# mikeferguson/ndt_2d

Measured on AMD Instinct MI355X. Metric: pose-candidates x beams scored per second, higher is better.
Workload: dtype f64

## Files before the change

### ndt_2d_amd/csrc/ndt2d_device_fn.h

```cpp
#ifndef NDT2D_DEVICE_FN_H_
#define NDT2D_DEVICE_FN_H_

#include <hip/hip_runtime.h>
#include <math.h>

#include "ndt2d_kernels.h"

namespace ndt2d
{

constexpr int kWave = 64;
constexpr int kRecord = 12;
constexpr double kNoIndex = 1.0e308;
constexpr double kPadCoord = -1.0e300;

template <bool POW2>
__device__ __forceinline__ uint32_t cell_index(const GridDesc & g, double px, double py)
{
  const double tx = px - g.origin_x;
  const double ty = py - g.origin_y;
  double fx, fy;
  if (POW2)
  {
    fx = tx * g.inv_cell_size;
// ... 8 lines not shown
                      (fy < static_cast<double>(g.size_y));
  const uint32_t gx = static_cast<uint32_t>(fx);
  const uint32_t gy = static_cast<uint32_t>(fy);
  return inside ? gy * g.size_x + gx : g.ncell;
}

__device__ __forceinline__ double record_exponent(double mx, double my, double h00,
                                                  double h01, double h11, double px, double py)
{
  const double q0 = px - mx;
  const double q1 = py - my;
  const double r0 = q0 * h00 + q1 * h01;
  const double r1 = q0 * h01 + q1 * h11;
  return r0 * q0 + r1 * q1;
}

__device__ __forceinline__ double record_likelihood(double mx, double my, double h00,
                                                    double h01, double h11, double px,
                                                    double py)
{
  return exp(record_exponent(mx, my, h00, h01, h11, px, py));
}

__device__ __forceinline__ double fma3(double a, double b, double c)
{
  double d;
  asm("v_fma_f64 %0, %1, %2, %3" : "=v"(d) : "v"(a), "v"(b), "v"(c));
  return d;
}
#ifndef NDT2D_EXP_SCALAR_CONSTANTS
#define NDT2D_EXP_SCALAR_CONSTANTS 0
#endif
template <uint32_t HI, uint32_t LO>
__device__ __forceinline__ double fma3k(double a, double b)
{
  double d;
#if NDT2D_EXP_SCALAR_CONSTANTS
  uint32_t lo, hi;
  asm volatile("s_mov_b32 %0, %2\n\ts_mov_b32 %1, %3" : "=s"(lo), "=s"(hi) : "n"(LO), "n"(HI));
  const double c = __hiloint2double(static_cast<int>(hi), static_cast<int>(lo));
  asm("v_fma_f64 %0, %1, %2, %3" : "=v"(d) : "v"(a), "v"(b), "s"(c));
#else
  asm("v_fma_f64 %0, %1, %2, %3" : "=v"(d) : "v"(a), "v"(b), "v"(__hiloint2double(static_cast<int>(HI), static_cast<int>(LO))));
#endif
  return d;
}

__device__ __forceinline__ double exp_of_exponent(double x)
{
  asm("v_max_f64 %0, %1, %2" : "=v"(x) : "v"(x), "s"(-1000.0));
  const double n = rint(x * 1.4426950408889634);
  double r = fma(n, -0.6931471805599453, x);
  r = fma(n, -2.3190468138462996e-17, r);
  double p = fma3k<0x3e928af3u, 0xfca7ab0cu>(r, 0x1.ade156a5dcb37p-26);
  p = fma3k<0x3ec71deeu, 0x623fde64u>(r, p);
  p = fma3k<0x3efa0199u, 0x7c89e6b0u>(r, p);
  p = fma3k<0x3f2a01a0u, 0x14761f6eu>(r, p);
  p = fma3k<0x3f56c16cu, 0x1852b7b0u>(r, p);
  p = fma3k<0x3f811111u, 0x11122322u>(r, p);
  p = fma3k<0x3fa55555u, 0x555502a1u>(r, p);
  p = fma3k<0x3fc55555u, 0x55555511u>(r, p);
  p = fma3k<0x3fe00000u, 0x0000000bu>(r, p);
  asm("v_fma_f64 %0, %1, %2, 1.0" : "=v"(p) : "v"(r), "v"(p));
  asm("v_fma_f64 %0, %1, %2, 1.0" : "=v"(p) : "v"(r), "v"(p));
  return ldexp(p, static_cast<int>(n));
}

__device__ __forceinline__ bool wave_any(bool p)
{
  return __builtin_amdgcn_ballot_w64(p) != 0ull;
}

constexpr double kExpOverflowAbove = 0x1.62e42fefa39efp+9;

__device__ __forceinline__ double exp_score(double e)
{
  double r = exp_of_exponent(e);
  if (__builtin_expect(wave_any(!(e <= kExpOverflowAbove)), 0))
  {
    r = (e != e) ? e + e : (e > kExpOverflowAbove ? HUGE_VAL : r);
  }
  return r;
}

__device__ __forceinline__ double negligible_below(double s)
{
  const double from_sum =
// ... 179 lines not shown
```

### ndt_2d_amd/csrc/ndt2d_lane_fn.h

```cpp
#ifndef NDT2D_LANE_FN_H_
#define NDT2D_LANE_FN_H_

#include <cmath>

#include "ndt2d_device_fn.h"

namespace ndt2d
{

namespace
{

constexpr int kPatch = 8;
#ifndef NDT2D_LANE_UNROLL
#define NDT2D_LANE_UNROLL 8
#endif
constexpr int kUnroll = NDT2D_LANE_UNROLL;
constexpr double kFracScale = 65536.0;
constexpr int kMapStride = 256;
constexpr int kMaxMapCells = 256;
constexpr uint32_t kNearUnits = 4;
constexpr double kBoxMargin = 1.0 / 1024.0;
constexpr double kTwo24 = 16777216.0;
constexpr double kTwo52 = 4503599627370496.0;
// ... 193 lines not shown
  return kRankLead + (((ncell + 1u) * 2u + 15u) & ~15u);
}

#if defined(NDT2D_LANE_HIST) || defined(NDT2D_LANE_PATHS)
__device__ double * g_lane_hist = nullptr;
#endif
#ifdef NDT2D_LANE_PATHS
#define NDT2D_PATH(slot, amount)                                                              \
  do {                                                                                        \
    if (g_lane_hist != nullptr && (threadIdx.x & 63u) == 0) atomicAdd(g_lane_hist + (slot), static_cast<double>(amount)); \
  } while (0)
#else
#define NDT2D_PATH(slot, amount) do {} while (0)
#endif

struct LaneCtx
{
  uint32_t rank_address;
  uint32_t lds_cells_address;
  uint32_t sub_log2;
  uint32_t exact_index;
  uint32_t idx_bias;
  uint32_t size_x;
};

__device__ __forceinline__ uint32_t lds_byte_at(uint32_t address)
{
  typedef const __attribute__((address_space(3))) uint8_t * lds_byte_ptr;
  return *reinterpret_cast<lds_byte_ptr>(address);
}

__device__ __forceinline__ uint32_t lds_u16_at(uint32_t address)
{
  typedef const __attribute__((address_space(3))) uint16_t * lds_u16_ptr;
  return *reinterpret_cast<lds_u16_ptr>(address);
}

__device__ __forceinline__ uint64_t near_boundary(uint32_t v)
{
  uint64_t lanes;
  asm("v_cmp_gt_u16_e64 %0, 8, %1" : "=s"(lanes) : "v"(v));
  return lanes;
}

__device__ __forceinline__ uint2 lds_two_dwords_at(uint32_t address)
{
  typedef const __attribute__((address_space(3), aligned(4))) uint32_t * lds_u32_ptr;
// ... 32 lines not shown
}

struct SkipState
{
  double skip_below;
  uint32_t skip_level;
};

__device__ __forceinline__ SkipState skip_state(double sum, int32_t no_skip)
{
  SkipState s;
  if (no_skip)
  {
    s.skip_below = -HUGE_VAL;
    s.skip_level = 0;
    return s;
  }
  s.skip_below = negligible_below(sum);
  const int32_t l = static_cast<int32_t>(ceil(s.skip_below)) + 63;
  s.skip_level = static_cast<uint32_t>(min(max(l, 1), 63)) << 2;
  return s;
}

template <int U, bool POW2, bool LDS_RECORDS, bool SCALAR_ROWS = true, bool COMPACT = false>
__device__ __forceinline__ void lane_beams(const GridDesc & g, const LaneCtx & c,
                                           const double4 (&o)[U], double dx, double dy,
                                           double dxy, double & sum, SkipState & skip,
                                           int32_t no_skip)
{
  const double skip_below = skip.skip_below;
  const uint32_t skip_level = skip.skip_level;
  uint32_t lo[U], hi[U], m[U];
  uint32_t top = 0;
#pragma unroll
  for (int u = 0; u < U; ++u)
  {
    const double s = o[u].z + dxy;
    lo[u] = static_cast<uint32_t>(__double2loint(s));
    hi[u] = static_cast<uint32_t>(__double2hiint(s));
    m[u] = lds_byte_at(__builtin_amdgcn_perm(hi[u], lo[u], 0x0c0c0502u));
    top = max(top, m[u]);
  }
  NDT2D_PATH(U == 1 ? 210 : 202, U);
  if (wave_any(top >= skip_level))
  {
    NDT2D_PATH(203, 1);
    bool added = false;
    if (SCALAR_ROWS)
    {
#pragma unroll
      for (int u = 0; u < U; ++u) asm volatile("" : : "s"(o[u].x), "s"(o[u].y));
    }
#pragma unroll
    for (int u = 0; u < U; ++u)
    {
      const uint64_t live_mask = __builtin_amdgcn_ballot_w64(m[u] >= skip_level);
      if (live_mask != 0ull)
      {
        NDT2D_PATH(204, 1);
        const uint32_t fy = __builtin_amdgcn_perm(hi[u], lo[u], 0x0c0c0403u);
        const bool occ = (m[u] & 1u) != 0;
        const uint64_t near_mask =
          (near_boundary(lo[u]) | near_boundary(fy) | ((no_skip | c.exact_index) != 0 ? ~0ull : 0ull)) & live_mask;
        const uint64_t occ_lanes = __builtin_amdgcn_ballot_w64(occ);
        const uint64_t occ_mask = occ_lanes & live_mask;
#ifdef NDT2D_LANE_NO_EXACT
        if ((occ_mask | near_mask) == 0x1234567ull)
#else
        if ((occ_mask | near_mask) != 0ull)
#endif
        {
          NDT2D_PATH(205, 1);
          if (near_mask != 0ull) NDT2D_PATH(206, 1);
          const double px = o[u].x + dx;
          const double py = o[u].y + dy;
          uint32_t idx;
          if (near_mask != 0ull)
          {
            idx = cell_index<POW2>(g, px, py);
          }
          else
          {
            const uint32_t col = ((lo[u] >> 16) & 0xffu) >> c.sub_log2;
            const uint32_t row = ((hi[u] >> 8) & 0xffu) >> c.sub_log2;
            const uint32_t cell = __umul24(row, c.size_x) + (col - c.idx_bias);
            if (COMPACT)
            {
              asm("v_cndmask_b32 %0, -1, %1, %2" : "=v"(idx) : "v"(cell), "s"(occ_lanes));
            }
            else
            {
              idx = occ ? cell : g.ncell;
            }
          }
          if (COMPACT) idx = lds_u16_at(c.rank_address + 2u * idx);
          const double e = LDS_RECORDS ? lds_record_exponent(c.lds_cells_address, idx, px, py)
                                       : indexed_exponent<false>(g, nullptr, idx, px, py);
#ifdef NDT2D_LANE_HIST
          if (g_lane_hist != nullptr)
          {
            const uint64_t flagged = occ_mask | near_mask;
            const uint64_t needed = __builtin_amdgcn_ballot_w64(!(e < skip_below)) & flagged;
            if ((threadIdx.x & 63u) == 0)
            {
              atomicAdd(g_lane_hist + __popcll(flagged), 1.0);
              atomicAdd(g_lane_hist + 70 + __popcll(needed), 1.0);
              atomicAdd(g_lane_hist + (needed != 0ull ? 140 : 141), 1.0);
            }
          }
#endif
          if (wave_any(!(e < skip_below)))
          {
            NDT2D_PATH(207, 1);
            sum += exp_score(e);
            added = true;
          }
        }
      }
// ... 99 lines not shown
```

### ndt_2d_amd/csrc/ndt2d_match_lane.hip

```cpp
#include <cmath>
#include <cstdlib>

#include <type_traits>

#include "ndt2d_lane_fn.h"

namespace ndt2d
{

namespace
{

constexpr uint32_t kDynamicItemsFromBeams = 256;
constexpr int kLaneThreads = 1024;
constexpr int kLaneThreadsSmall = 256;
#ifndef NDT2D_LANE_THREADS_COMPACT
#define NDT2D_LANE_THREADS_COMPACT 768
#endif
constexpr int kLaneThreadsCompact = NDT2D_LANE_THREADS_COMPACT;
#define NDT2D_LANE_COMPACT_WAVES_PER_EU (NDT2D_LANE_THREADS_COMPACT / 128)

__global__ void __launch_bounds__(256) outer_table_kernel(const MatchArgs a, double4 * outer,
                                                          uint8_t * map_out, const LaneGeom geo)
{
  {
    const GridDesc & g = a.grid;
    const uint32_t n_map = static_cast<uint32_t>(kMapStride) * geo.map_h;
    for (uint32_t i = blockIdx.x * 256 + threadIdx.x; i < n_map; i += gridDim.x * 256)
    {
      const int32_t mx = static_cast<int32_t>(i & (kMapStride - 1));
      const int32_t my = static_cast<int32_t>(i >> 8);
      if (geo.block_log2 > 0)
      {
        const int32_t cells = 1 << geo.block_log2;
        map_out[i] = block_byte(g, mx * cells - geo.pad + geo.win_x0, my * cells - geo.pad + geo.win_y0, cells);
        continue;
      }
      const int32_t sub = 1 << geo.sub_log2;
      const int32_t cx = (mx >> geo.sub_log2) - geo.pad + geo.win_x0;
      const int32_t cy = (my >> geo.sub_log2) - geo.pad + geo.win_y0;
      map_out[i] = sub_cell_byte(g, cx, cy, mx & (sub - 1), my & (sub - 1), geo.sub_log2);
    }
  }

  if (blockIdx.x == 0 && threadIdx.x < kItemShards) a.next_item[threadIdx.x * kItemShardStride] = 0u;
  const uint64_t n = static_cast<uint64_t>(a.th_end - a.th_begin) * a.n_beams;
  for (uint64_t i = static_cast<uint64_t>(blockIdx.x) * 256 + threadIdx.x; i < n;
       i += static_cast<uint64_t>(gridDim.x) * 256)
  {
    const uint32_t t = static_cast<uint32_t>(i / a.n_beams);
    const uint32_t b = static_cast<uint32_t>(i - static_cast<uint64_t>(t) * a.n_beams);
    const uint32_t ith = a.th_begin + t * a.th_stride;
    const double ct = a.cos_th[ith];
    const double st = a.sin_th[ith];
    const double2 p = reinterpret_cast<const double2 *>(a.beams_xy)[b];
    double4 o;
    o.x = p.x * ct - p.y * st + a.pose_x;
    o.y = p.x * st + p.y * ct + a.pose_y;
    double kx = ((o.x - a.grid.origin_x) * a.grid.inv_cell_size + (geo.pad - geo.win_x0)) * geo.unit_scale;
    double ky = ((o.y - a.grid.origin_y) * a.grid.inv_cell_size + (geo.pad - geo.win_y0)) * geo.unit_scale;
    kx = !(kx >= geo.k_min) ? geo.k_min : (kx > geo.k_max_x ? geo.k_max_x : kx);
    ky = !(ky >= geo.k_min) ? geo.k_min : (ky > geo.k_max_y ? geo.k_max_y : ky);
    o.z = kTwo52 + (rint(ky) * kTwo24 + rint(kx)) + kNearBias;
    o.w = 0.0;
    outer[i] = o;
  }
}

__device__ __forceinline__ void item_place(uint32_t item, uint32_t patches, uint32_t patches_1d,
                                           uint32_t th_mid, uint32_t & t, uint32_t & pxi, uint32_t & pyi)
{
  const uint32_t rank = item / patches;
  const uint32_t p = item - rank * patches;
  t = (rank & 1u) ? th_mid + (rank + 1u) / 2u : th_mid - rank / 2u;
  pxi = p / patches_1d;
  pyi = p - pxi * patches_1d;
}

__device__ __forceinline__ double packed_offset(double dx, double dy, double inv_scaled)
{
  return rint(dy * inv_scaled) * kTwo24 + rint(dx * inv_scaled);
}

__device__ __forceinline__ double no_index_here()
{
  static_assert(kNoIndex == 1.0e308, "the literal below is 1.0e308");
  uint32_t lo, hi;
  asm volatile("v_mov_b32 %0, 0x85ebc8a0\n\tv_mov_b32 %1, 0x7fe1ccf3" : "=v"(lo), "=v"(hi));
  return __hiloint2double(static_cast<int>(hi), static_cast<int>(lo));
}

template <int THREADS, bool POW2, bool LDS_RECORDS, bool DYNAMIC_ITEMS, bool COMPACT, bool PARTS = false>
__device__ __forceinline__ void match_lane_body(
  const MatchArgs & a, const double4 * __restrict__ outer, const uint8_t * __restrict__ map_image,
  const LaneGeom & geo)
{
  extern __shared__ __align__(16) double lds[];
  const GridDesc & g = a.grid;
#if defined(NDT2D_LANE_HIST) || defined(NDT2D_LANE_PATHS)
  if (blockIdx.x == 0 && threadIdx.x == 0) g_lane_hist = a.scores;
#endif
  uint8_t * lds_map = reinterpret_cast<uint8_t *>(lds);
  const uint32_t map_bytes = static_cast<uint32_t>(geo.map_h) * kMapStride;
  const uint32_t rank_bytes = COMPACT ? compact_rank_bytes(g.ncell) : 0u;
  double * lds_cells = lds + (map_bytes + rank_bytes) / sizeof(double);

  if (COMPACT)
  {
    const uint4 * src_rank = reinterpret_cast<const uint4 *>(g.cell_rank);
    uint4 * dst_rank = reinterpret_cast<uint4 *>(lds_map + map_bytes + kRankLead);
    for (uint32_t i = threadIdx.x; i < (rank_bytes - kRankLead) / 16; i += THREADS) dst_rank[i] = src_rank[i];
    if (threadIdx.x == 0)
    {
      reinterpret_cast<uint16_t *>(lds_map + map_bytes + kRankLead)[-1] = static_cast<uint16_t>(g.n_occ);
    }
    const uint32_t n2 = (g.n_occ + 1) * kCellDoubles / 2;
    const double2 * src = reinterpret_cast<const double2 *>(g.compact_records);
// ... 5 lines not shown
    stage_grid_to_lds(g, lds_cells);
  }
  {
    const uint32_t n16 = static_cast<uint32_t>(kMapStride) * geo.map_h / 16;
    const uint4 * src = reinterpret_cast<const uint4 *>(map_image);
    uint4 * dst = reinterpret_cast<uint4 *>(lds_map);
    for (uint32_t i = threadIdx.x; i < n16; i += THREADS) dst[i] = src[i];
  }
  __syncthreads();

#ifdef NDT2D_LANE_TRACE
  const unsigned long long trace_t0 = wall_clock64();
  unsigned long long trace_last = trace_t0, trace_max = 0, trace_last_start = trace_t0;
  uint32_t trace_items = 0, trace_prev_item = 0, trace_flagged = 0;
#endif
  LaneCtx c;
  c.rank_address = map_bytes + (COMPACT ? kRankLead : 0u);
  c.lds_cells_address = map_bytes + rank_bytes;
  c.sub_log2 = static_cast<uint32_t>(geo.sub_log2);
  c.exact_index = geo.block_log2 > 0 ? 1u : 0u;
  c.idx_bias = static_cast<uint32_t>(geo.pad - geo.win_y0) * g.size_x +
               static_cast<uint32_t>(geo.pad - geo.win_x0);
  c.size_x = g.size_x;

  const uint32_t lane = threadIdx.x & (kWave - 1);
  const uint32_t wave = __builtin_amdgcn_readfirstlane(threadIdx.x >> 6);
  const uint32_t n_lin = a.n_lin;
  const uint32_t patches_1d = (n_lin + kPatch - 1) / kPatch;
  const uint32_t patches = patches_1d * patches_1d;
  const uint32_t n_items = (a.th_end - a.th_begin) * patches * (PARTS ? a.beam_parts : 1u);
  constexpr uint32_t kLaneWaves = THREADS / kWave;
  const uint32_t n_workers = gridDim.x * kLaneWaves;
  const uint32_t worker = wave * gridDim.x + blockIdx.x;
  const uint64_t per_theta = static_cast<uint64_t>(n_lin) * n_lin;
  const uint32_t th_mid = (a.th_end - a.th_begin - 1u) / 2u;
  const uint32_t home_shard = blockIdx.x % kItemShards;
  const double inv_scaled = geo.inv_scaled;

  double best_s = 0.0;
  double best_i = kNoIndex;
  double acc[10];
#pragma unroll
  for (int k = 0; k < 10; ++k) acc[k] = 0.0;
  for (uint32_t item = worker; item < n_items;)
  {
    uint32_t t, pxi, pyi;
// ... 4 lines not shown
      if (trace_items > 0 && a.scores != nullptr && lane == 0)
      {
        a.scores[5 * 8192 + 150000 + trace_prev_item] = static_cast<double>(now - trace_last);
        a.scores[5 * 8192 + 300000 + trace_prev_item] = static_cast<double>(trace_flagged);
      }
      trace_flagged = 0;
      trace_prev_item = item;
      trace_last = now;
      trace_last_start = now;
      ++trace_items;
      if (a.scores != nullptr && lane == 0) a.scores[5 * 8192 + item] = static_cast<double>(now);
    }
#endif
    const uint32_t whole_item = PARTS ? item / a.beam_parts : item;
    const uint32_t part = PARTS ? item - whole_item * a.beam_parts : 0u;
    item_place(whole_item, patches, patches_1d, th_mid, t, pxi, pyi);
    uint32_t lane_here = lane;
    asm volatile("" : "+v"(lane_here));
    const uint32_t ix = pxi * kPatch + (lane_here >> 3);
    const uint32_t iy = pyi * kPatch + (lane_here & 7);
    const double dx = a.dlin[min(ix, n_lin - 1)];
    const double dy = a.dlin[min(iy, n_lin - 1)];
    const double dxy = packed_offset(dx, dy, inv_scaled);
    const double4 * __restrict__ row = outer + static_cast<size_t>(t) * a.n_beams;

    double sum = 0.0;
    SkipState skip = skip_state(0.0, geo.no_skip);
    NDT2D_PATH(200, 1);
    const double dxy_corner = __hiloint2double(__builtin_amdgcn_readfirstlane(__double2hiint(dxy)),
                                               __builtin_amdgcn_readfirstlane(__double2loint(dxy)));
    const uint32_t beams_begin = PARTS ? part * a.part_beams : 0u;
    const uint32_t beams_end = PARTS ? min(beams_begin + a.part_beams, a.n_beams) : a.n_beams;
    for (uint32_t b0 = beams_begin; b0 < beams_end; b0 += kWave)
    {
      uint64_t can_score = ~0ull;
      if (geo.box_span >= 0)
      {
        const double k = row[min(b0 + lane, a.n_beams - 1u)].z;
        can_score = __builtin_amdgcn_ballot_w64(patch_can_score(k + dxy_corner, geo.box_span));
        NDT2D_PATH(201, 1);
      }
#ifdef NDT2D_LANE_TRACE
      trace_flagged += static_cast<uint32_t>(__popcll(can_score));
#endif
      const uint32_t chunk_end = min(b0 + static_cast<uint32_t>(kWave), beams_end);
      uint32_t b = b0;
      for (; b + kUnroll <= chunk_end; b += kUnroll, can_score >>= kUnroll)
      {
        if ((can_score & ((1ull << kUnroll) - 1ull)) == 0ull) continue;
        double4 o[kUnroll];
#pragma unroll
        for (int u = 0; u < kUnroll; ++u) o[u] = row[b + u];
        __builtin_amdgcn_s_setprio(3);
        lane_beams<kUnroll, POW2, LDS_RECORDS, true, COMPACT>(g, c, o, dx, dy, dxy, sum, skip, geo.no_skip);
        __builtin_amdgcn_s_setprio(0);
      }
      for (; b < chunk_end; ++b, can_score >>= 1)
      {
        if ((can_score & 1ull) == 0ull) continue;
        const double4 one[1] = {row[b]};
        lane_beams<1, POW2, LDS_RECORDS, true, COMPACT>(g, c, one, dx, dy, dxy, sum, skip, geo.no_skip);
      }
    }

    if (PARTS)
    {
      a.part_sums[static_cast<size_t>(item) * kWave + lane] = sum;
      uint32_t next = n_items;
      if (lane == kWave - 1)
      {
        for (uint32_t tried = 0; tried < kItemShards && next >= n_items; ++tried)
        {
          const uint32_t shard = (home_shard + tried) % kItemShards;
          const uint32_t k = atomicAdd(a.next_item + shard * kItemShardStride, 1u);
          const uint64_t candidate = static_cast<uint64_t>(n_workers) + static_cast<uint64_t>(k) * kItemShards + shard;
          if (candidate < n_items) next = static_cast<uint32_t>(candidate);
        }
      }
      item = static_cast<uint32_t>(__builtin_amdgcn_readlane(static_cast<int>(next), kWave - 1));
      continue;
    }
    uint32_t lane_again = lane;
    asm volatile("" : "+v"(lane_again));
    const uint32_t ix_e = pxi * kPatch + (lane_again >> 3);
// ... 80 lines not shown
    a.scores[5 * worker + 2] = static_cast<double>(trace_items);
    a.scores[5 * worker + 3] = static_cast<double>(trace_max);
    a.scores[5 * worker + 4] = static_cast<double>(trace_last_start);
  }
#endif
  if (!DYNAMIC_ITEMS)
  {
    wave_best_to_last_lane(best_s, best_i);
#pragma unroll
    for (int k = 0; k < 10; ++k) acc[k] = wave_sum_to_last_lane(acc[k]);
    if (lane == kWave - 1)
    {
      double * out = a.partials + static_cast<size_t>(worker) * kRecord;
      out[0] = best_s;
      out[1] = best_i;
#pragma unroll
      for (int k = 0; k < 10; ++k) out[2 + k] = acc[k];
    }
  }
}

template <int THREADS, bool POW2, bool LDS_RECORDS, bool DYNAMIC_ITEMS>
__global__ void __launch_bounds__(THREADS) match_lane_kernel(
  const MatchArgs a, const double4 * __restrict__ outer, const uint8_t * __restrict__ map_image,
  const LaneGeom geo)
{
  match_lane_body<THREADS, POW2, LDS_RECORDS, DYNAMIC_ITEMS, false>(a, outer, map_image, geo);
}

__global__ void __launch_bounds__(kLaneThreadsCompact) __attribute__((amdgpu_waves_per_eu(NDT2D_LANE_COMPACT_WAVES_PER_EU)))
match_lane_compact_kernel(const MatchArgs a, const double4 * __restrict__ outer,
                          const uint8_t * __restrict__ map_image, const LaneGeom geo)
{
  match_lane_body<kLaneThreadsCompact, true, true, true, true>(a, outer, map_image, geo);
}

template <bool POW2>
__global__ void __launch_bounds__(kLaneThreadsCompact) __attribute__((amdgpu_waves_per_eu(NDT2D_LANE_COMPACT_WAVES_PER_EU)))
match_lane_gather6_kernel(const MatchArgs a, const double4 * __restrict__ outer,
                          const uint8_t * __restrict__ map_image, const LaneGeom geo)
{
  match_lane_body<kLaneThreadsCompact, POW2, false, true, false>(a, outer, map_image, geo);
}

__global__ void __launch_bounds__(kLaneThreadsCompact) __attribute__((amdgpu_waves_per_eu(NDT2D_LANE_COMPACT_WAVES_PER_EU)))
match_lane_compact_parts_kernel(const MatchArgs a, const double4 * __restrict__ outer,
                                const uint8_t * __restrict__ map_image, const LaneGeom geo)
{
  match_lane_body<kLaneThreadsCompact, true, true, true, true, true>(a, outer, map_image, geo);
}

template <bool POW2>
__global__ void __launch_bounds__(kLaneThreadsCompact) __attribute__((amdgpu_waves_per_eu(NDT2D_LANE_COMPACT_WAVES_PER_EU)))
match_lane_gather6_parts_kernel(const MatchArgs a, const double4 * __restrict__ outer,
                                const uint8_t * __restrict__ map_image, const LaneGeom geo)
{
  match_lane_body<kLaneThreadsCompact, POW2, false, true, false, true>(a, outer, map_image, geo);
}

__global__ void __launch_bounds__(256) match_lane_combine_kernel(const MatchArgs a)
{
  const uint32_t lane = threadIdx.x & (kWave - 1);
  const uint32_t n_lin = a.n_lin;
  const uint32_t patches_1d = (n_lin + kPatch - 1) / kPatch;
  const uint32_t patches = patches_1d * patches_1d;
  const uint32_t n_items = (a.th_end - a.th_begin) * patches;
  const uint32_t item = blockIdx.x * 4u + (threadIdx.x >> 6);
  if (item >= n_items) return;
  const uint32_t th_mid = (a.th_end - a.th_begin - 1u) / 2u;
  uint32_t t, pxi, pyi;
  item_place(item, patches, patches_1d, th_mid, t, pxi, pyi);
  const uint32_t ix = pxi * kPatch + (lane >> 3);
  const uint32_t iy = pyi * kPatch + (lane & 7);
  const bool valid = (ix < n_lin) & (iy < n_lin);
  const double * p = a.part_sums + static_cast<size_t>(item) * a.beam_parts * kWave + lane;
  double sum = p[0];
  for (uint32_t j = 1; j < a.beam_parts; ++j) sum += p[static_cast<size_t>(j) * kWave];
// ... 81 lines not shown
  {
    const long long v = std::atoll(env);
    if (v > 0 && static_cast<uint64_t>(v) <= kMaxLaneItems) slab_items = static_cast<uint64_t>(v);
  }
  uint64_t th = slab_items / per_theta;
  if (th < 1) th = 1;
  const uint64_t at_least = (th_total + kMaxLaneSlabs - 1) / kMaxLaneSlabs;
  if (th < at_least) th = at_least;
  if (th > th_total) th = th_total;
  if (th * per_theta > kMaxLaneItems) return false;
  *slab_th = static_cast<uint32_t>(th);
  *n_slabs = static_cast<uint32_t>((th_total + th - 1) / th);
  return true;
}

size_t match_lane_outer_doubles(const MatchArgs & args)
{
  uint32_t slab_th = args.th_end - args.th_begin, n_slabs = 1;
  (void)lane_slabs(args, &slab_th, &n_slabs);
  uint32_t part_beams = 0;
  const uint32_t parts = lane_beam_parts(args, &part_beams);
  const uint64_t p1 = (args.n_lin + kPatch - 1) / kPatch;
  const size_t part_sums = parts > 1 ? static_cast<size_t>(slab_th) * p1 * p1 * parts * kWave : 0;
  return static_cast<size_t>(slab_th) * args.n_beams * 4 +
         static_cast<size_t>(kMapStride) * kMaxMapCells / sizeof(double) + part_sums;
}

bool match_lane_supported(const MatchArgs & args, size_t lds_per_block)
{
  LaneGeom geo;
  size_t map_bytes = 0;
  if (args.grid.occ_bits == nullptr || !lane_geometry(args, lds_per_block, &geo, &map_bytes)) return false;
  uint32_t slab_th = 0, n_slabs = 0;
  return map_bytes <= lds_per_block && lane_slabs(args, &slab_th, &n_slabs) &&
         args.grid.size_x < (1u << 24) && args.grid.ncell < (1u << 24);
}

hipError_t launch_match_lane(const MatchArgs & args_in, double * outer, double * workspace,
                             uint32_t max_workers, int cus, size_t lds_per_block, bool no_skip,
                             hipStream_t stream, hipEvent_t ev_after_pre_kernel,
                             uint32_t * n_workers_out, int * records_mode_out, uint32_t * parts_out)
{
  MatchArgs args = args_in;
  args.partials = workspace;
  LaneGeom geo;
  size_t map_bytes = 0;
  if (!lane_geometry(args, lds_per_block, &geo, &map_bytes)) return hipErrorInvalidValue;
  geo.no_skip = no_skip ? 1 : 0;
  {
    static const bool pretest = [] {
      const char * v = std::getenv("NDT2D_LANE_PRETEST");
      return v == nullptr || v[0] != '0';
    }();
    if (no_skip || !pretest) geo.box_span = -1;
  }
  const bool dynamic_items = args.n_beams >= kDynamicItemsFromBeams;
  const uint32_t p1 = (args.n_lin + kPatch - 1) / kPatch;
  const uint64_t n_items = static_cast<uint64_t>(args.th_end - args.th_begin) * p1 * p1;

  const uint64_t n_outer = static_cast<uint64_t>(args.th_end - args.th_begin) * args.n_beams;
  uint32_t oblocks = static_cast<uint32_t>((n_outer + 255) / 256);
  if (oblocks > 4096) oblocks = 4096;
  if (oblocks < 64) oblocks = 64;
  uint8_t * map_image = reinterpret_cast<uint8_t *>(outer + n_outer * 4);
  uint32_t part_beams = 0;
  uint32_t beam_parts = dynamic_items ? lane_beam_parts(args, &part_beams) : 1u;
  args.part_sums = outer + n_outer * 4 + static_cast<size_t>(kMapStride) * kMaxMapCells / sizeof(double);

  const char * knob_rec = std::getenv("NDT2D_LANE_RECORDS");
  const bool lds_records = lane_records_in_lds(args, map_bytes, lds_per_block) &&
                           !(knob_rec != nullptr && knob_rec[0] == 'g');
  size_t lds_bytes =
    map_bytes +
    (lds_records ? static_cast<size_t>(args.grid.ncell + 1) * kCellDoubles * sizeof(double) : 0);
  const size_t compact_bytes =
    compact_rank_bytes(args.grid.ncell) +
    (static_cast<size_t>(args.grid.n_occ) + 1) * kCellDoubles * sizeof(double);
  const char * knob = std::getenv("NDT2D_LANE_COMPACT");
  const bool compact_possible = dynamic_items && pow2_grid(args) && lds_records && args.grid.n_occ > 0 &&
                                args.grid.compact_records != nullptr &&
                                2 * (map_bytes + compact_bytes) <= lds_per_block &&
                                !(knob != nullptr && knob[0] == '0');
  const char * knob6 = std::getenv("NDT2D_LANE_GATHER6");
  const bool gather6_possible = dynamic_items && !lds_records && 2 * map_bytes <= lds_per_block &&
                                !(knob6 != nullptr && knob6[0] == '0');
  if (!(compact_possible || gather6_possible)) beam_parts = 1;
  args.beam_parts = beam_parts;
  args.part_beams = part_beams;
  const uint64_t n_sub_items = n_items * beam_parts;

  const bool small = beam_parts == 1 && n_items <= static_cast<uint64_t>(cus) * (kLaneThreadsSmall / kWave);
  const uint32_t waves_per_block = (small ? kLaneThreadsSmall : kLaneThreads) / kWave;
  uint32_t blocks = static_cast<uint32_t>((n_items + waves_per_block - 1) / waves_per_block);
  uint32_t max_blocks = static_cast<uint32_t>(cus);
  if (max_blocks * waves_per_block > max_workers) max_blocks = max_workers / waves_per_block;
  if (blocks > max_blocks) blocks = max_blocks;
  if (blocks == 0) blocks = 1;
  const bool compact = !small && compact_possible;
  const bool gather6 = !compact && !small && gather6_possible;
  if (records_mode_out != nullptr)
  {
    *records_mode_out = (compact ? 2 : (lds_records ? 1 : 0)) | (geo.block_log2 > 0 ? 4 : 0);
  }
  if (compact || gather6)
  {
    lds_bytes = compact ? map_bytes + compact_bytes : map_bytes;
    const uint32_t wpb = kLaneThreadsCompact / kWave;
    blocks = static_cast<uint32_t>((n_sub_items + wpb - 1) / wpb);
    uint32_t cap = 2 * static_cast<uint32_t>(cus);
    if (cap * wpb > max_workers) cap = max_workers / wpb;
    if (blocks > cap) blocks = cap;
    if (blocks == 0) blocks = 1;
  }
  hipLaunchKernelGGL(outer_table_kernel, dim3(oblocks), dim3(256), 0, stream, args,
                     reinterpret_cast<double4 *>(outer), map_image, geo);
  hipError_t e = hipGetLastError();
  if (e != hipSuccess) return e;
  if (ev_after_pre_kernel != nullptr)
  {
    e = hipEventRecord(ev_after_pre_kernel, stream);
    if (e != hipSuccess) return e;
  }
  auto launch = [&](auto kernel, int threads) -> hipError_t {
    const hipError_t e2 = prepare_absolute_lds_kernel(reinterpret_cast<const void *>(kernel), lds_bytes);
    if (e2 != hipSuccess) return e2;
    hipLaunchKernelGGL(kernel, dim3(blocks), dim3(threads), lds_bytes, stream, args,
                       reinterpret_cast<const double4 *>(outer),
                       static_cast<const uint8_t *>(map_image), geo);
    return hipGetLastError();
  };
  const bool pow2 = args.grid.pow2 != 0;
  auto pick = [&](auto threads_tag) -> hipError_t {
    constexpr int T = decltype(threads_tag)::value;
    auto with_items = [&](auto dyn_tag) -> hipError_t {
      constexpr bool D = decltype(dyn_tag)::value;
      return lds_records ? (pow2 ? launch(match_lane_kernel<T, true, true, D>, T)
                                 : launch(match_lane_kernel<T, false, true, D>, T))
                         : (pow2 ? launch(match_lane_kernel<T, true, false, D>, T)
                                 : launch(match_lane_kernel<T, false, false, D>, T));
    };
    return dynamic_items ? with_items(std::true_type{}) : with_items(std::false_type{});
  };
  if (beam_parts > 1)
  {
    e = compact ? launch(match_lane_compact_parts_kernel, kLaneThreadsCompact)
                : (pow2 ? launch(match_lane_gather6_parts_kernel<true>, kLaneThreadsCompact)
                        : launch(match_lane_gather6_parts_kernel<false>, kLaneThreadsCompact));
    if (e == hipSuccess)
    {
      hipLaunchKernelGGL(match_lane_combine_kernel, dim3(static_cast<uint32_t>((n_items + 3) / 4)), dim3(256),
// ... 28 lines not shown
```

### ndt_2d_amd/csrc/ndt2d_match_small.hip

```cpp
#include <cstdio>
#include <cstdlib>
#include <cstring>
#include <type_traits>

#include "ndt2d_lane_fn.h"

namespace ndt2d
{

namespace
{

constexpr int kSmallMaxWaves = 16;
constexpr int kSmallUnroll = 4;
constexpr uint32_t kSmallMaxBeams = 2048;
constexpr uint32_t kRowDoubles = 3;

struct SmallPlan
{
  uint32_t patches_per_block;
  uint32_t chunks;
  uint32_t chunk_beams;
  uint32_t blocks_per_theta;
  uint32_t need_w;
// ... 275 lines not shown
      const double oy = p.x * st + p.y * ct + a.pose_y;
      double kx = ((ox - g.origin_x) * g.inv_cell_size + (geo.pad - geo.win_x0)) * geo.unit_scale;
      double ky = ((oy - g.origin_y) * g.inv_cell_size + (geo.pad - geo.win_y0)) * geo.unit_scale;
      kx = !(kx >= geo.k_min) ? geo.k_min : (kx > geo.k_max_x ? geo.k_max_x : kx);
      ky = !(ky >= geo.k_min) ? geo.k_min : (ky > geo.k_max_y ? geo.k_max_y : ky);
      rows[kRowDoubles * b + 0] = ox;
      rows[kRowDoubles * b + 1] = oy;
      rows[kRowDoubles * b + 2] = kTwo52 + (rint(ky) * kTwo24 + rint(kx)) + kNearBias;
    }
  }
  __syncthreads();
#ifdef NDT2D_SMALL_TRACE
  const unsigned long long t_setup = __builtin_readcyclecounter();
#endif

  LaneCtx c;
  c.rank_address = map_bytes + (COMPACT ? kRankLead : 0u);
  c.lds_cells_address = map_bytes + rank_bytes;
  c.sub_log2 = 0;
  c.exact_index = geo.block_log2 > 0 ? 1u : 0u;
  c.idx_bias = static_cast<uint32_t>(geo.pad - geo.win_y0) * g.size_x +
               static_cast<uint32_t>(geo.pad - geo.win_x0);
  c.size_x = g.size_x;

  const uint32_t lane = threadIdx.x & (kWave - 1);
  const uint32_t wave = __builtin_amdgcn_readfirstlane(threadIdx.x >> 6);
  const uint32_t slot = wave / plan.chunks;
  const uint32_t chunk = wave - slot * plan.chunks;
  const uint32_t n_lin = a.n_lin;
  const uint32_t tile = first_patch + slot;
  const bool active = slot < plan.patches_per_block && tile < plan.tiles;

  uint32_t ix, iy;
  if (plan.linear)
  {
    const uint32_t f = (active ? tile : 0u) * kWave + lane;
    ix = f / n_lin;
    iy = f - ix * n_lin;
  }
  else
  {
    const uint32_t patches_1d = (n_lin + kPatch - 1) / kPatch;
    const uint32_t pxi = active ? tile / patches_1d : 0;
    const uint32_t pyi = active ? tile - pxi * patches_1d : 0;
    ix = pxi * kPatch + (lane >> 3);
    iy = pyi * kPatch + (lane & 7);
  }
  const bool valid = active & (ix < n_lin) & (iy < n_lin);
  const double dx = table(3, min(ix, n_lin - 1));
  const double dy = table(3, min(iy, n_lin - 1));

  if (active)
  {
    const double inv_scaled = g.inv_cell_size * geo.unit_scale;
    const double dxy = rint(dy * inv_scaled) * kTwo24 + rint(dx * inv_scaled);
    auto row_at = [&](uint32_t beam) -> double4 {
      const double * r = rows + kRowDoubles * beam;
      double4 o;
      o.x = r[0];
      o.y = r[1];
      o.z = r[2];
      o.w = 0.0;
      return o;
    };
    double sum = 0.0;
    SkipState skip = skip_state(0.0, geo.no_skip);
    for (uint32_t b = chunk * kSmallUnroll; b < a.n_beams; b += plan.chunks * kSmallUnroll)
    {
      if (b + kSmallUnroll <= a.n_beams)
      {
        double4 o[kSmallUnroll];
#pragma unroll
        for (int u = 0; u < kSmallUnroll; ++u) o[u] = row_at(b + u);
        lane_beams<kSmallUnroll, POW2, COMPACT, false, COMPACT>(g, c, o, dx, dy, dxy, sum, skip, geo.no_skip);
      }
      else
      {
        for (uint32_t t = b; t < a.n_beams; ++t)
        {
          const double4 one[1] = {row_at(t)};
          lane_beams<1, POW2, COMPACT, false, COMPACT>(g, c, one, dx, dy, dxy, sum, skip, geo.no_skip);
        }
      }
    }
    partials[wave * kWave + lane] = sum;
  }
#ifdef NDT2D_SMALL_TRACE
  const unsigned long long t_main = __builtin_readcyclecounter();
#endif
  __syncthreads();
#ifdef NDT2D_SMALL_TRACE
  const unsigned long long t_barrier = __builtin_readcyclecounter();
#endif

  if (active && chunk == 0)
  {
    const double * mine = partials + static_cast<size_t>(slot) * plan.chunks * kWave + lane;
    double sum = mine[0];
    for (uint32_t j = 1; j < plan.chunks; ++j) sum += mine[j * kWave];

    double best_s = 0.0;
    double best_i = kNoIndex;
    double acc[10];
#pragma unroll
// ... 289 lines not shown
```

Measured before the change: 3034 billion.

## Split beam table into key and xy planes with lazy point fetch

Replaces the interleaved double4 beam table with a padded struct-of-arrays layout: a plane of packed cell keys and a separate plane of xy coordinates. The lane kernel loads only the keys up front and fetches xy coordinates only when some beam in the group survives the skip test, and it iterates over set bits of the can-score mask instead of scanning every group. The exp polynomial is emitted as one asm block, and the per-call near-mask select and rank-address add are precomputed or fused. This aims to cut wasted memory traffic and loop overhead, at the cost of a padded table and more complex indexing.

```diff
diff --git a/ndt_2d_amd/csrc/ndt2d_device_fn.h b/ndt_2d_amd/csrc/ndt2d_device_fn.h
--- a/ndt_2d_amd/csrc/ndt2d_device_fn.h
+++ b/ndt_2d_amd/csrc/ndt2d_device_fn.h
@@ -54,37 +54,27 @@
   return exp(record_exponent(mx, my, h00, h01, h11, px, py));
 }
 
-__device__ __forceinline__ double fma3(double a, double b, double c)
-{
-  double d;
-  asm("v_fma_f64 %0, %1, %2, %3" : "=v"(d) : "v"(a), "v"(b), "v"(c));
-  return d;
-}
 #ifndef NDT2D_EXP_SCALAR_CONSTANTS
 #define NDT2D_EXP_SCALAR_CONSTANTS 0
 #endif
+#if NDT2D_EXP_SCALAR_CONSTANTS
 template <uint32_t HI, uint32_t LO>
 __device__ __forceinline__ double fma3k(double a, double b)
 {
   double d;
-#if NDT2D_EXP_SCALAR_CONSTANTS
   uint32_t lo, hi;
   asm volatile("s_mov_b32 %0, %2\n\ts_mov_b32 %1, %3" : "=s"(lo), "=s"(hi) : "n"(LO), "n"(HI));
   const double c = __hiloint2double(static_cast<int>(hi), static_cast<int>(lo));
   asm("v_fma_f64 %0, %1, %2, %3" : "=v"(d) : "v"(a), "v"(b), "s"(c));
-#else
-  asm("v_fma_f64 %0, %1, %2, %3" : "=v"(d) : "v"(a), "v"(b), "v"(__hiloint2double(static_cast<int>(HI), static_cast<int>(LO))));
-#endif
   return d;
 }
-
-__device__ __forceinline__ double exp_of_exponent(double x)
-{
-  asm("v_max_f64 %0, %1, %2" : "=v"(x) : "v"(x), "s"(-1000.0));
-  const double n = rint(x * 1.4426950408889634);
-  double r = fma(n, -0.6931471805599453, x);
-  r = fma(n, -2.3190468138462996e-17, r);
-  double p = fma3k<0x3e928af3u, 0xfca7ab0cu>(r, 0x1.ade156a5dcb37p-26);
+#endif
+
+__device__ __forceinline__ double exp_polynomial(double r)
+{
+  double p;
+#if NDT2D_EXP_SCALAR_CONSTANTS
+  p = fma3k<0x3e928af3u, 0xfca7ab0cu>(r, 0x1.ade156a5dcb37p-26);
   p = fma3k<0x3ec71deeu, 0x623fde64u>(r, p);
   p = fma3k<0x3efa0199u, 0x7c89e6b0u>(r, p);
   p = fma3k<0x3f2a01a0u, 0x14761f6eu>(r, p);
@@ -93,8 +83,41 @@
   p = fma3k<0x3fa55555u, 0x555502a1u>(r, p);
   p = fma3k<0x3fc55555u, 0x55555511u>(r, p);
   p = fma3k<0x3fe00000u, 0x0000000bu>(r, p);
-  asm("v_fma_f64 %0, %1, %2, 1.0" : "=v"(p) : "v"(r), "v"(p));
-  asm("v_fma_f64 %0, %1, %2, 1.0" : "=v"(p) : "v"(r), "v"(p));
+  asm("v_fma_f64 %0, %1, %2, 1.0\n\tv_fma_f64 %0, %1, %0, 1.0" : "=&v"(p) : "v"(r), "v"(p));
+#else
+  asm("v_fma_f64 %0, %1, %2, %3\n\t"
+      "v_fma_f64 %0, %1, %0, %4\n\t"
+      "v_fma_f64 %0, %1, %0, %5\n\t"
+      "v_fma_f64 %0, %1, %0, %6\n\t"
+      "v_fma_f64 %0, %1, %0, %7\n\t"
+      "v_fma_f64 %0, %1, %0, %8\n\t"
+      "v_fma_f64 %0, %1, %0, %9\n\t"
+      "v_fma_f64 %0, %1, %0, %10\n\t"
+      "v_fma_f64 %0, %1, %0, %11\n\t"
+      "v_fma_f64 %0, %1, %0, 1.0\n\t"
+      "v_fma_f64 %0, %1, %0, 1.0"
+      : "=&v"(p)
+      : "v"(r), "v"(0x1.ade156a5dcb37p-26),
+        "v"(0x1.28af3fca7ab0cp-22),
+        "v"(0x1.71dee623fde64p-19),
+        "v"(0x1.a01997c89e6b0p-16),
+        "v"(0x1.a01a014761f6ep-13),
+        "v"(0x1.6c16c1852b7b0p-10),
+        "v"(0x1.1111111122322p-7),
+        "v"(0x1.55555555502a1p-5),
+        "v"(0x1.5555555555511p-3),
+        "v"(0x1.000000000000bp-1));
+#endif
+  return p;
+}
+
+__device__ __forceinline__ double exp_of_exponent(double x)
+{
+  asm("v_max_f64 %0, %1, %2" : "=v"(x) : "v"(x), "s"(-1000.0));
+  const double n = rint(x * 1.4426950408889634);
+  double r = fma(n, -0.6931471805599453, x);
+  r = fma(n, -2.3190468138462996e-17, r);
+  const double p = exp_polynomial(r);
   return ldexp(p, static_cast<int>(n));
 }
 
diff --git a/ndt_2d_amd/csrc/ndt2d_lane_fn.h b/ndt_2d_amd/csrc/ndt2d_lane_fn.h
--- a/ndt_2d_amd/csrc/ndt2d_lane_fn.h
+++ b/ndt_2d_amd/csrc/ndt2d_lane_fn.h
@@ -239,7 +239,13 @@
   uint32_t exact_index;
   uint32_t idx_bias;
   uint32_t size_x;
+  uint64_t always_near;
 };
+
+__device__ __forceinline__ uint64_t lane_always_near(int32_t no_skip, uint32_t exact_index)
+{
+  return 0ull - static_cast<uint64_t>(min(static_cast<uint32_t>(no_skip) | exact_index, 1u));
+}
 
 __device__ __forceinline__ uint32_t lds_byte_at(uint32_t address)
 {
@@ -318,10 +324,49 @@
   return s;
 }
 
-template <int U, bool POW2, bool LDS_RECORDS, bool SCALAR_ROWS = true, bool COMPACT = false>
+template <int U>
+struct LoadedPoints
+{
+  double2 p[U];
+  __device__ __forceinline__ void fetch(double2 (&xy)[U]) const
+  {
+#pragma unroll
+    for (int u = 0; u < U; ++u) xy[u] = p[u];
+  }
+};
+
+typedef double lane_double8 __attribute__((ext_vector_type(8)));
+template <int U>
+struct UniformPoints
+{
+  const double * __restrict__ at;
+  __device__ __forceinline__ void fetch(double2 (&xy)[U]) const
+  {
+    if constexpr (U == 8)
+    {
+      const lane_double8 a = *reinterpret_cast<const lane_double8 *>(at);
+      const lane_double8 b = *reinterpret_cast<const lane_double8 *>(at + 8);
+#pragma unroll
+      for (int u = 0; u < 4; ++u)
+      {
+        xy[u] = make_double2(a[2 * u], a[2 * u + 1]);
+        xy[4 + u] = make_double2(b[2 * u], b[2 * u + 1]);
+      }
+    }
+    else
+    {
+#pragma unroll
+      for (int u = 0; u < U; ++u) xy[u] = make_double2(at[2 * u], at[2 * u + 1]);
+    }
+#pragma unroll
+    for (int u = 0; u < U; ++u) asm volatile("" : : "s"(xy[u].x), "s"(xy[u].y));
+  }
+};
+
+template <int U, bool POW2, bool LDS_RECORDS, bool COMPACT, class Points>
 __device__ __forceinline__ void lane_beams(const GridDesc & g, const LaneCtx & c,
-                                           const double4 (&o)[U], double dx, double dy,
-                                           double dxy, double & sum, SkipState & skip,
+                                           const double (&k)[U], const Points & points, double dx,
+                                           double dy, double dxy, double & sum, SkipState & skip,
                                            int32_t no_skip)
 {
   const double skip_below = skip.skip_below;
@@ -331,7 +376,7 @@
 #pragma unroll
   for (int u = 0; u < U; ++u)
   {
-    const double s = o[u].z + dxy;
+    const double s = k[u] + dxy;
     lo[u] = static_cast<uint32_t>(__double2loint(s));
     hi[u] = static_cast<uint32_t>(__double2hiint(s));
     m[u] = lds_byte_at(__builtin_amdgcn_perm(hi[u], lo[u], 0x0c0c0502u));
@@ -342,11 +387,8 @@
   {
     NDT2D_PATH(203, 1);
     bool added = false;
-    if (SCALAR_ROWS)
-    {
-#pragma unroll
-      for (int u = 0; u < U; ++u) asm volatile("" : : "s"(o[u].x), "s"(o[u].y));
-    }
+    double2 xy[U];
+    points.fetch(xy);
 #pragma unroll
     for (int u = 0; u < U; ++u)
     {
@@ -357,7 +399,7 @@
         const uint32_t fy = __builtin_amdgcn_perm(hi[u], lo[u], 0x0c0c0403u);
         const bool occ = (m[u] & 1u) != 0;
         const uint64_t near_mask =
-          (near_boundary(lo[u]) | near_boundary(fy) | ((no_skip | c.exact_index) != 0 ? ~0ull : 0ull)) & live_mask;
+          (near_boundary(lo[u]) | near_boundary(fy) | c.always_near) & live_mask;
         const uint64_t occ_lanes = __builtin_amdgcn_ballot_w64(occ);
         const uint64_t occ_mask = occ_lanes & live_mask;
 #ifdef NDT2D_LANE_NO_EXACT
@@ -368,12 +410,13 @@
         {
           NDT2D_PATH(205, 1);
           if (near_mask != 0ull) NDT2D_PATH(206, 1);
-          const double px = o[u].x + dx;
-          const double py = o[u].y + dy;
+          const double px = xy[u].x + dx;
+          const double py = xy[u].y + dy;
           uint32_t idx;
           if (near_mask != 0ull)
           {
             idx = cell_index<POW2>(g, px, py);
+            if (COMPACT) idx = c.rank_address + 2u * idx;
           }
           else
           {
@@ -382,14 +425,15 @@
             const uint32_t cell = __umul24(row, c.size_x) + (col - c.idx_bias);
             if (COMPACT)
             {
-              asm("v_cndmask_b32 %0, -1, %1, %2" : "=v"(idx) : "v"(cell), "s"(occ_lanes));
+              asm("v_cndmask_b32 %0, -1, %1, %2\n\tv_lshl_add_u32 %0, %0, 1, %3"
+                  : "=v"(idx) : "v"(cell), "s"(occ_lanes), "s"(c.rank_address));
             }
             else
             {
               idx = occ ? cell : g.ncell;
             }
           }
-          if (COMPACT) idx = lds_u16_at(c.rank_address + 2u * idx);
+          if (COMPACT) idx = lds_u16_at(idx);
           const double e = LDS_RECORDS ? lds_record_exponent(c.lds_cells_address, idx, px, py)
                                        : indexed_exponent<false>(g, nullptr, idx, px, py);
 #ifdef NDT2D_LANE_HIST
diff --git a/ndt_2d_amd/csrc/ndt2d_match_lane.hip b/ndt_2d_amd/csrc/ndt2d_match_lane.hip
--- a/ndt_2d_amd/csrc/ndt2d_match_lane.hip
+++ b/ndt_2d_amd/csrc/ndt2d_match_lane.hip
@@ -20,7 +20,17 @@
 constexpr int kLaneThreadsCompact = NDT2D_LANE_THREADS_COMPACT;
 #define NDT2D_LANE_COMPACT_WAVES_PER_EU (NDT2D_LANE_THREADS_COMPACT / 128)
 
-__global__ void __launch_bounds__(256) outer_table_kernel(const MatchArgs a, double4 * outer,
+constexpr uint32_t kTableGroup = kUnroll > 8 ? kUnroll : 8;
+__host__ __device__ inline uint32_t table_stride(uint32_t n_beams)
+{
+  return (n_beams + kTableGroup - 1u) / kTableGroup * kTableGroup;
+}
+__host__ __device__ inline size_t table_doubles(uint32_t n_th, uint32_t n_beams)
+{
+  return static_cast<size_t>(n_th) * table_stride(n_beams) * 3;
+}
+
+__global__ void __launch_bounds__(256) outer_table_kernel(const MatchArgs a, double * outer,
                                                           uint8_t * map_out, const LaneGeom geo)
 {
   {
@@ -44,26 +54,34 @@
   }
 
   if (blockIdx.x == 0 && threadIdx.x < kItemShards) a.next_item[threadIdx.x * kItemShardStride] = 0u;
-  const uint64_t n = static_cast<uint64_t>(a.th_end - a.th_begin) * a.n_beams;
+  const uint32_t stride = table_stride(a.n_beams);
+  const uint64_t n = static_cast<uint64_t>(a.th_end - a.th_begin) * stride;
+  double * const k_plane = outer;
+  double2 * const xy_plane = reinterpret_cast<double2 *>(outer + n);
   for (uint64_t i = static_cast<uint64_t>(blockIdx.x) * 256 + threadIdx.x; i < n;
        i += static_cast<uint64_t>(gridDim.x) * 256)
   {
-    const uint32_t t = static_cast<uint32_t>(i / a.n_beams);
-    const uint32_t b = static_cast<uint32_t>(i - static_cast<uint64_t>(t) * a.n_beams);
+    const uint32_t t = static_cast<uint32_t>(i / stride);
+    const uint32_t b = static_cast<uint32_t>(i - static_cast<uint64_t>(t) * stride);
+    if (b >= a.n_beams)
+    {
+      k_plane[i] = 0.0;
+      xy_plane[i] = make_double2(0.0, 0.0);
+      continue;
+    }
     const uint32_t ith = a.th_begin + t * a.th_stride;
     const double ct = a.cos_th[ith];
     const double st = a.sin_th[ith];
     const double2 p = reinterpret_cast<const double2 *>(a.beams_xy)[b];
-    double4 o;
+    double2 o;
     o.x = p.x * ct - p.y * st + a.pose_x;
     o.y = p.x * st + p.y * ct + a.pose_y;
     double kx = ((o.x - a.grid.origin_x) * a.grid.inv_cell_size + (geo.pad - geo.win_x0)) * geo.unit_scale;
     double ky = ((o.y - a.grid.origin_y) * a.grid.inv_cell_size + (geo.pad - geo.win_y0)) * geo.unit_scale;
     kx = !(kx >= geo.k_min) ? geo.k_min : (kx > geo.k_max_x ? geo.k_max_x : kx);
     ky = !(ky >= geo.k_min) ? geo.k_min : (ky > geo.k_max_y ? geo.k_max_y : ky);
-    o.z = kTwo52 + (rint(ky) * kTwo24 + rint(kx)) + kNearBias;
-    o.w = 0.0;
-    outer[i] = o;
+    k_plane[i] = kTwo52 + (rint(ky) * kTwo24 + rint(kx)) + kNearBias;
+    xy_plane[i] = o;
   }
 }
 
@@ -92,7 +110,7 @@
 
 template <int THREADS, bool POW2, bool LDS_RECORDS, bool DYNAMIC_ITEMS, bool COMPACT, bool PARTS = false>
 __device__ __forceinline__ void match_lane_body(
-  const MatchArgs & a, const double4 * __restrict__ outer, const uint8_t * __restrict__ map_image,
+  const MatchArgs & a, const double * __restrict__ outer, const uint8_t * __restrict__ map_image,
   const LaneGeom & geo)
 {
   extern __shared__ __align__(16) double lds[];
@@ -144,6 +162,10 @@
   c.idx_bias = static_cast<uint32_t>(geo.pad - geo.win_y0) * g.size_x +
                static_cast<uint32_t>(geo.pad - geo.win_x0);
   c.size_x = g.size_x;
+  c.always_near = lane_always_near(geo.no_skip, c.exact_index);
+  const uint32_t table_row = table_stride(a.n_beams);
+  const double * __restrict__ const k_plane = outer;
+  const double * __restrict__ const xy_plane = outer + static_cast<size_t>(a.th_end - a.th_begin) * table_row;
 
   const uint32_t lane = threadIdx.x & (kWave - 1);
   const uint32_t wave = __builtin_amdgcn_readfirstlane(threadIdx.x >> 6);
@@ -194,7 +216,8 @@
     const double dx = a.dlin[min(ix, n_lin - 1)];
     const double dy = a.dlin[min(iy, n_lin - 1)];
     const double dxy = packed_offset(dx, dy, inv_scaled);
-    const double4 * __restrict__ row = outer + static_cast<size_t>(t) * a.n_beams;
+    const double * __restrict__ krow = k_plane + static_cast<size_t>(t) * table_row;
+    const double * __restrict__ xyrow = xy_plane + static_cast<size_t>(t) * table_row * 2;
 
     double sum = 0.0;
     SkipState skip = skip_state(0.0, geo.no_skip);
@@ -203,35 +226,55 @@
                                                __builtin_amdgcn_readfirstlane(__double2loint(dxy)));
     const uint32_t beams_begin = PARTS ? part * a.part_beams : 0u;
     const uint32_t beams_end = PARTS ? min(beams_begin + a.part_beams, a.n_beams) : a.n_beams;
+    constexpr uint64_t kGroupBits = (1ull << kUnroll) - 1ull;
     for (uint32_t b0 = beams_begin; b0 < beams_end; b0 += kWave)
     {
       uint64_t can_score = ~0ull;
       if (geo.box_span >= 0)
       {
-        const double k = row[min(b0 + lane, a.n_beams - 1u)].z;
+        const double k = krow[min(b0 + lane, a.n_beams - 1u)];
         can_score = __builtin_amdgcn_ballot_w64(patch_can_score(k + dxy_corner, geo.box_span));
         NDT2D_PATH(201, 1);
       }
 #ifdef NDT2D_LANE_TRACE
       trace_flagged += static_cast<uint32_t>(__popcll(can_score));
 #endif
-      const uint32_t chunk_end = min(b0 + static_cast<uint32_t>(kWave), beams_end);
-      uint32_t b = b0;
-      for (; b + kUnroll <= chunk_end; b += kUnroll, can_score >>= kUnroll)
-      {
-        if ((can_score & ((1ull << kUnroll) - 1ull)) == 0ull) continue;
-        double4 o[kUnroll];
-#pragma unroll
-        for (int u = 0; u < kUnroll; ++u) o[u] = row[b + u];
+      const uint32_t n_here = min(static_cast<uint32_t>(kWave), beams_end - b0);
+      const uint32_t n_whole = n_here & ~static_cast<uint32_t>(kUnroll - 1);
+      uint64_t groups = n_whole == static_cast<uint32_t>(kWave) ? can_score : (can_score & ((1ull << n_whole) - 1ull));
+      while (groups != 0ull)
+      {
+        const uint32_t first = static_cast<uint32_t>(__builtin_ctzll(groups)) & ~static_cast<uint32_t>(kUnroll - 1);
+        groups &= ~(kGroupBits << first);
+        const uint32_t b = b0 + first;
+        double k[kUnroll];
+        if constexpr (kUnroll == 8)
+        {
+          const lane_double8 k8 = *reinterpret_cast<const lane_double8 *>(krow + b);
+#pragma unroll
+          for (int u = 0; u < kUnroll; ++u) k[u] = k8[u];
+        }
+        else
+        {
+#pragma unroll
+          for (int u = 0; u < kUnroll; ++u) k[u] = krow[b + u];
+        }
+        const UniformPoints<kUnroll> points = {xyrow + 2 * b};
         __builtin_amdgcn_s_setprio(3);
-        lane_beams<kUnroll, POW2, LDS_RECORDS, true, COMPACT>(g, c, o, dx, dy, dxy, sum, skip, geo.no_skip);
+        lane_beams<kUnroll, POW2, LDS_RECORDS, COMPACT>(g, c, k, points, dx, dy, dxy, sum, skip, geo.no_skip);
         __builtin_amdgcn_s_setprio(0);
       }
-      for (; b < chunk_end; ++b, can_score >>= 1)
-      {
-        if ((can_score & 1ull) == 0ull) continue;
-        const double4 one[1] = {row[b]};
-        lane_beams<1, POW2, LDS_RECORDS, true, COMPACT>(g, c, one, dx, dy, dxy, sum, skip, geo.no_skip);
+      if (n_whole != n_here)
+      {
+        uint64_t tail = (can_score >> n_whole) & ((1ull << (n_here - n_whole)) - 1ull);
+        while (tail != 0ull)
+        {
+          const uint32_t b = b0 + n_whole + static_cast<uint32_t>(__builtin_ctzll(tail));
+          tail &= tail - 1ull;
+          const double one[1] = {krow[b]};
+          const UniformPoints<1> point = {xyrow + 2 * b};
+          lane_beams<1, POW2, LDS_RECORDS, COMPACT>(g, c, one, point, dx, dy, dxy, sum, skip, geo.no_skip);
+        }
       }
     }
 
@@ -358,14 +401,14 @@
 
 template <int THREADS, bool POW2, bool LDS_RECORDS, bool DYNAMIC_ITEMS>
 __global__ void __launch_bounds__(THREADS) match_lane_kernel(
-  const MatchArgs a, const double4 * __restrict__ outer, const uint8_t * __restrict__ map_image,
+  const MatchArgs a, const double * __restrict__ outer, const uint8_t * __restrict__ map_image,
   const LaneGeom geo)
 {
   match_lane_body<THREADS, POW2, LDS_RECORDS, DYNAMIC_ITEMS, false>(a, outer, map_image, geo);
 }
 
 __global__ void __launch_bounds__(kLaneThreadsCompact) __attribute__((amdgpu_waves_per_eu(NDT2D_LANE_COMPACT_WAVES_PER_EU)))
-match_lane_compact_kernel(const MatchArgs a, const double4 * __restrict__ outer,
+match_lane_compact_kernel(const MatchArgs a, const double * __restrict__ outer,
                           const uint8_t * __restrict__ map_image, const LaneGeom geo)
 {
   match_lane_body<kLaneThreadsCompact, true, true, true, true>(a, outer, map_image, geo);
@@ -373,14 +416,14 @@
 
 template <bool POW2>
 __global__ void __launch_bounds__(kLaneThreadsCompact) __attribute__((amdgpu_waves_per_eu(NDT2D_LANE_COMPACT_WAVES_PER_EU)))
-match_lane_gather6_kernel(const MatchArgs a, const double4 * __restrict__ outer,
+match_lane_gather6_kernel(const MatchArgs a, const double * __restrict__ outer,
                           const uint8_t * __restrict__ map_image, const LaneGeom geo)
 {
   match_lane_body<kLaneThreadsCompact, POW2, false, true, false>(a, outer, map_image, geo);
 }
 
 __global__ void __launch_bounds__(kLaneThreadsCompact) __attribute__((amdgpu_waves_per_eu(NDT2D_LANE_COMPACT_WAVES_PER_EU)))
-match_lane_compact_parts_kernel(const MatchArgs a, const double4 * __restrict__ outer,
+match_lane_compact_parts_kernel(const MatchArgs a, const double * __restrict__ outer,
                                 const uint8_t * __restrict__ map_image, const LaneGeom geo)
 {
   match_lane_body<kLaneThreadsCompact, true, true, true, true, true>(a, outer, map_image, geo);
@@ -388,7 +431,7 @@
 
 template <bool POW2>
 __global__ void __launch_bounds__(kLaneThreadsCompact) __attribute__((amdgpu_waves_per_eu(NDT2D_LANE_COMPACT_WAVES_PER_EU)))
-match_lane_gather6_parts_kernel(const MatchArgs a, const double4 * __restrict__ outer,
+match_lane_gather6_parts_kernel(const MatchArgs a, const double * __restrict__ outer,
                                 const uint8_t * __restrict__ map_image, const LaneGeom geo)
 {
   match_lane_body<kLaneThreadsCompact, POW2, false, true, false, true>(a, outer, map_image, geo);
@@ -516,7 +559,7 @@
   const uint32_t parts = lane_beam_parts(args, &part_beams);
   const uint64_t p1 = (args.n_lin + kPatch - 1) / kPatch;
   const size_t part_sums = parts > 1 ? static_cast<size_t>(slab_th) * p1 * p1 * parts * kWave : 0;
-  return static_cast<size_t>(slab_th) * args.n_beams * 4 +
+  return table_doubles(slab_th, args.n_beams) +
          static_cast<size_t>(kMapStride) * kMaxMapCells / sizeof(double) + part_sums;
 }
 
@@ -552,14 +595,15 @@
   const uint32_t p1 = (args.n_lin + kPatch - 1) / kPatch;
   const uint64_t n_items = static_cast<uint64_t>(args.th_end - args.th_begin) * p1 * p1;
 
-  const uint64_t n_outer = static_cast<uint64_t>(args.th_end - args.th_begin) * args.n_beams;
+  const size_t n_table = table_doubles(args.th_end - args.th_begin, args.n_beams);
+  const uint64_t n_outer = n_table / 3;
   uint32_t oblocks = static_cast<uint32_t>((n_outer + 255) / 256);
   if (oblocks > 4096) oblocks = 4096;
   if (oblocks < 64) oblocks = 64;
-  uint8_t * map_image = reinterpret_cast<uint8_t *>(outer + n_outer * 4);
+  uint8_t * map_image = reinterpret_cast<uint8_t *>(outer + n_table);
   uint32_t part_beams = 0;
   uint32_t beam_parts = dynamic_items ? lane_beam_parts(args, &part_beams) : 1u;
-  args.part_sums = outer + n_outer * 4 + static_cast<size_t>(kMapStride) * kMaxMapCells / sizeof(double);
+  args.part_sums = outer + n_table + static_cast<size_t>(kMapStride) * kMaxMapCells / sizeof(double);
 
   const char * knob_rec = std::getenv("NDT2D_LANE_RECORDS");
   const bool lds_records = lane_records_in_lds(args, map_bytes, lds_per_block) &&
@@ -606,8 +650,7 @@
     if (blocks > cap) blocks = cap;
     if (blocks == 0) blocks = 1;
   }
-  hipLaunchKernelGGL(outer_table_kernel, dim3(oblocks), dim3(256), 0, stream, args,
-                     reinterpret_cast<double4 *>(outer), map_image, geo);
+  hipLaunchKernelGGL(outer_table_kernel, dim3(oblocks), dim3(256), 0, stream, args, outer, map_image, geo);
   hipError_t e = hipGetLastError();
   if (e != hipSuccess) return e;
   if (ev_after_pre_kernel != nullptr)
@@ -619,7 +662,7 @@
     const hipError_t e2 = prepare_absolute_lds_kernel(reinterpret_cast<const void *>(kernel), lds_bytes);
     if (e2 != hipSuccess) return e2;
     hipLaunchKernelGGL(kernel, dim3(blocks), dim3(threads), lds_bytes, stream, args,
-                       reinterpret_cast<const double4 *>(outer),
+                       static_cast<const double *>(outer),
                        static_cast<const uint8_t *>(map_image), geo);
     return hipGetLastError();
   };
diff --git a/ndt_2d_amd/csrc/ndt2d_match_small.hip b/ndt_2d_amd/csrc/ndt2d_match_small.hip
--- a/ndt_2d_amd/csrc/ndt2d_match_small.hip
+++ b/ndt_2d_amd/csrc/ndt2d_match_small.hip
@@ -321,6 +321,7 @@
   c.idx_bias = static_cast<uint32_t>(geo.pad - geo.win_y0) * g.size_x +
                static_cast<uint32_t>(geo.pad - geo.win_x0);
   c.size_x = g.size_x;
+  c.always_near = lane_always_near(geo.no_skip, c.exact_index);
 
   const uint32_t lane = threadIdx.x & (kWave - 1);
   const uint32_t wave = __builtin_amdgcn_readfirstlane(threadIdx.x >> 6);
@@ -353,14 +354,11 @@
   {
     const double inv_scaled = g.inv_cell_size * geo.unit_scale;
     const double dxy = rint(dy * inv_scaled) * kTwo24 + rint(dx * inv_scaled);
-    auto row_at = [&](uint32_t beam) -> double4 {
+    auto row_at = [&](uint32_t beam, double & k, double2 & xy) {
       const double * r = rows + kRowDoubles * beam;
-      double4 o;
-      o.x = r[0];
-      o.y = r[1];
-      o.z = r[2];
-      o.w = 0.0;
-      return o;
+      xy.x = r[0];
+      xy.y = r[1];
+      k = r[2];
     };
     double sum = 0.0;
     SkipState skip = skip_state(0.0, geo.no_skip);
@@ -368,17 +366,20 @@
     {
       if (b + kSmallUnroll <= a.n_beams)
       {
-        double4 o[kSmallUnroll];
-#pragma unroll
-        for (int u = 0; u < kSmallUnroll; ++u) o[u] = row_at(b + u);
-        lane_beams<kSmallUnroll, POW2, COMPACT, false, COMPACT>(g, c, o, dx, dy, dxy, sum, skip, geo.no_skip);
+        double k[kSmallUnroll];
+        LoadedPoints<kSmallUnroll> o;
+#pragma unroll
+        for (int u = 0; u < kSmallUnroll; ++u) row_at(b + u, k[u], o.p[u]);
+        lane_beams<kSmallUnroll, POW2, COMPACT, COMPACT>(g, c, k, o, dx, dy, dxy, sum, skip, geo.no_skip);
       }
       else
       {
         for (uint32_t t = b; t < a.n_beams; ++t)
         {
-          const double4 one[1] = {row_at(t)};
-          lane_beams<1, POW2, COMPACT, false, COMPACT>(g, c, one, dx, dy, dxy, sum, skip, geo.no_skip);
+          double k[1];
+          LoadedPoints<1> one;
+          row_at(t, k[0], one.p[0]);
+          lane_beams<1, POW2, COMPACT, COMPACT>(g, c, k, one, dx, dy, dxy, sum, skip, geo.no_skip);
         }
       }
     }
```

New measurement: 3052 billion, median of 6. No clear change (+0.6%).
